# OpenPPL/ppq

Hardware: AMD Instinct MI355X
Metric: calibration samples/sec (RuntimeCalibrationPass, KL 2048-bin, ResNet-50 INT8) (higher is better)
Workload: dtype f32; 1 GPU; ResNet-50 topology (53 Conv + 1 Gemm, BN folded, seeded He init), RuntimeCalibrationPass kl 2048 bins, per-tensor INT8 activations, per-channel INT8 weights, 279 batches x 32 x 3x224x224 per GPU; samples=8928, batch=32, observed_tensors=72, rccl_ranks=1, async_observe=False, cache_params=False, channels_last=False, fuse_params=True, batch_observations=True, reuse_activations=False, replayed_batches=0, hip_graph=auto, graph_replays=0, miopen_find=False

## Files before the change

include/ppq_hip.h:

```cpp
#ifndef PPQ_HIP_H_
#define PPQ_HIP_H_

#include <stdint.h>

#ifdef __cplusplus
extern "C" {
#endif

typedef enum {
    PPQHIP_OK = 0,
    PPQHIP_ERR_INVALID_VALUE = -1,
    PPQHIP_ERR_UNSUPPORTED = -2,
    PPQHIP_ERR_HIP = -3
} ppqhip_status;

#define PPQHIP_ABI_VERSION 4

const char* ppqhip_last_error(void);
int ppqhip_version(void);
int ppqhip_device_arch(char* buf, int n);

int ppqhip_fq_linear_t(const float* x, const float* scale, const float* offset, float* out,
                       int64_t n, int clip_min, int clip_max, int rounding, void* stream);

// ... 191 lines not shown
                         int64_t n, int64_t num_channel, int64_t elem_per_channel,
                         int clip_min, int clip_max, int rounding, void* stream);
int ppqhip_rounding_loss_bwd(const float* x, const float* dy, const float* scale,
                             const float* offset, float* dx, int64_t n, int64_t num_channel,
                             int64_t elem_per_channel, int clip_min, int clip_max, int rounding,
                             void* stream);

int ppqhip_bias_act(float* y, const float* bias, int64_t n, int64_t num_channel, int64_t elem_per_channel,
                    int relu, void* stream);
int ppqhip_bias_add_act(float* a, const float* bias_a, float* b, const float* bias_b, float* out,
                        int64_t n, int64_t num_channel, int64_t elem_per_channel, int relu, void* stream);

#define PPQHIP_NOT_FUSED 1
int ppqhip_bias_act_stats(float* y, const float* bias, int64_t n, int64_t num_channel, int64_t elem_per_channel,
                          int relu, float* slots_y, void* stream);
int ppqhip_bias_add_act_stats(float* a, const float* bias_a, float* b, const float* bias_b, float* out,
                              int64_t n, int64_t num_channel, int64_t elem_per_channel, int relu,
                              float* slots_a, float* slots_b, float* slots_out, void* stream);

#define PPQHIP_ELIDE_A 1
#define PPQHIP_ELIDE_B 2
int ppqhip_bias_add_act_stats2(float* a, const float* bias_a, float* b, const float* bias_b, float* out,
                               int64_t n, int64_t num_channel, int64_t elem_per_channel, int relu,
                               float* slots_a, float* slots_b, float* slots_out, int elide, void* stream);

int ppqhip_bias_act_hist(float* y, const float* bias, int64_t n, int64_t num_channel, int64_t elem_per_channel,
                         int relu, int32_t* rows_y, float p0_y, float p1_y, int64_t num_bins, int asymmetric,
                         int clip_outliers, void* stream);
int ppqhip_bias_add_act_hist(float* a, const float* bias_a, float* b, const float* bias_b, float* out,
                             int64_t n, int64_t num_channel, int64_t elem_per_channel, int relu,
                             int32_t* rows_a, float p0_a, float p1_a, int32_t* rows_b, float p0_b, float p1_b,
                             int32_t* rows_out, float p0_out, float p1_out, int64_t num_bins, int asymmetric,
                             int clip_outliers, int elide, void* stream);

typedef struct ppqhip_adaround_job {
    const float* w;
    const float* v;
    const float* scale;
    const float* offset;
    float* out;
    const float* dy;
    int64_t n, num_channel, elem_per_channel;
    int32_t qmin, qmax;
} ppqhip_adaround_job;
int ppqhip_adaround_fwd_multi(const ppqhip_adaround_job* jobs, int num_jobs, void* stream);
int ppqhip_adaround_bwd_multi(const ppqhip_adaround_job* jobs, int num_jobs, const float* reg, void* stream);

typedef struct ppqhip_roundtune_job {
    const float* w;
    const float* r;
    const float* scale;
    const float* offset;
    float* out;
    int64_t n, num_channel, elem_per_channel;
    int32_t qmin, qmax;
} ppqhip_roundtune_job;
int ppqhip_roundtune_fwd_multi(const ppqhip_roundtune_job* jobs, int num_jobs, void* stream);

typedef struct ppqhip_fetch_rows_job {
    const float* x;
    const int32_t* index;
    float* out;
    int64_t rows, row_len, count;
} ppqhip_fetch_rows_job;
int ppqhip_fetch_rows_multi(const ppqhip_fetch_rows_job* jobs, int num_jobs, void* stream);
typedef struct ppqhip_measure_rows_job {
// ... 169 lines not shown
```

ppq_amd/_lib.py:

```python
import ctypes
import os

_HERE = os.path.dirname(os.path.abspath(__file__))
LIB_PATH = os.path.join(_HERE, 'libppq_hip.so')

c_f32p = ctypes.c_void_p
c_i32p = ctypes.c_void_p
c_f64p = ctypes.c_void_p
c_i64 = ctypes.c_int64
c_int = ctypes.c_int
c_flt = ctypes.c_float
c_vp = ctypes.c_void_p

ABI_VERSION = 4


NOT_FUSED = 1


class ProfEntry(ctypes.Structure):
    _fields_ = [('name', ctypes.c_char * 48), ('launches', ctypes.c_int64),
                ('total_ms', ctypes.c_double), ('total_bytes', ctypes.c_double)]


PROTOTYPES = {
    'ppqhip_last_error': (ctypes.c_char_p, []),
    'ppqhip_version': (c_int, []),
    'ppqhip_device_arch': (c_int, [ctypes.c_char_p, c_int]),
    'ppqhip_fq_linear_t': (c_int, [c_f32p, c_f32p, c_f32p, c_f32p, c_i64, c_int, c_int, c_int, c_vp]),
    'ppqhip_fq_linear_c': (c_int, [c_f32p, c_f32p, c_f32p, c_f32p, c_i64, c_i64, c_i64, c_int, c_int, c_int, c_vp]),
    'ppqhip_to_int_t': (c_int, [c_f32p, c_f32p, c_f32p, c_vp, c_i64, c_int, c_int, c_int, c_int, c_vp]),
    'ppqhip_to_int_c': (c_int, [c_f32p, c_f32p, c_f32p, c_vp, c_i64, c_i64, c_i64, c_int, c_int, c_int, c_int, c_vp]),
    'ppqhip_fq_linear_t_bwd': (c_int, [c_f32p, c_f32p, c_f32p, c_f32p, c_f32p, c_f32p, c_i64, c_int, c_int, c_int,
                                       c_vp]),
    'ppqhip_fq_linear_c_bwd': (c_int, [c_f32p, c_f32p, c_f32p, c_f32p, c_f32p, c_f32p, c_i64, c_i64, c_i64, c_int,
                                       c_int, c_int, c_vp]),
    'ppqhip_fq_linear_c_bwd_multi': (c_int, [c_vp, c_int, c_int, c_vp]),
    'ppqhip_fq_linear_t_bwd_partials': (c_i64, [c_i64]),
    'ppqhip_fq_linear_t_bwd_main': (c_int, [c_f32p, c_f32p, c_f32p, c_f32p, c_f32p, c_f32p, c_i64, c_int, c_int, c_int, c_vp]),
    'ppqhip_lsq_finish_multi': (c_int, [c_vp, c_int, c_vp]),
    'ppqhip_bias_act': (c_int, [c_f32p, c_f32p, c_i64, c_i64, c_i64, c_int, c_vp]),
    'ppqhip_bias_add_act': (c_int, [c_f32p, c_f32p, c_f32p, c_f32p, c_f32p, c_i64, c_i64, c_i64, c_int, c_vp]),
    'ppqhip_bias_act_stats': (c_int, [c_f32p, c_f32p, c_i64, c_i64, c_i64, c_int, c_f32p, c_vp]),
    'ppqhip_bias_add_act_stats': (c_int, [c_f32p, c_f32p, c_f32p, c_f32p, c_f32p, c_i64, c_i64, c_i64, c_int, c_f32p, c_f32p,
                                          c_f32p, c_vp]),
    'ppqhip_bias_add_act_stats2': (c_int, [c_f32p, c_f32p, c_f32p, c_f32p, c_f32p, c_i64, c_i64, c_i64, c_int, c_f32p, c_f32p,
                                           c_f32p, c_int, c_vp]),
    'ppqhip_bias_act_hist': (c_int, [c_f32p, c_f32p, c_i64, c_i64, c_i64, c_int, c_i32p, c_flt, c_flt, c_i64, c_int, c_int, c_vp]),
    'ppqhip_bias_add_act_hist': (c_int, [c_f32p, c_f32p, c_f32p, c_f32p, c_f32p, c_i64, c_i64, c_i64, c_int,
                                         c_i32p, c_flt, c_flt, c_i32p, c_flt, c_flt, c_i32p, c_flt, c_flt, c_i64, c_int, c_int,
                                         c_int, c_vp]),
    'ppqhip_fq_float_t': (c_int, [c_f32p, c_f32p, c_f32p, c_f32p, c_i64, c_int, c_int, c_flt, c_flt, c_int, c_vp]),
    'ppqhip_fq_float_c': (c_int, [c_f32p, c_f32p, c_f32p, c_f32p, c_i64, c_i64, c_i64, c_int, c_int, c_flt, c_flt,
                                  c_int, c_vp]),
    'ppqhip_fq_float_c_bwd': (c_int, [c_f32p, c_f32p, c_f32p, c_f32p, c_f32p, c_f32p, c_i64, c_i64, c_i64, c_int,
                                      c_int, c_flt, c_flt, c_int, c_vp]),
    'ppqhip_hist_workspace_bytes': (c_i64, [c_i64, c_i64]),
    'ppqhip_hist_sym_t': (c_int, [c_f32p, c_i64, c_flt, c_int, c_i32p, c_i64, c_vp, c_vp]),
    'ppqhip_hist_asym_t': (c_int, [c_f32p, c_i64, c_flt, c_flt, c_int, c_i32p, c_i64, c_vp, c_vp]),
    'ppqhip_hist_sym_c': (c_int, [c_f32p, c_i64, c_i64, c_i64, c_flt, c_int, c_i32p, c_i64, c_vp]),
    'ppqhip_hist_sym_c_scales': (c_int, [c_f32p, c_i64, c_i64, c_i64, c_f32p, c_int, c_i32p, c_i64, c_vp]),
    'ppqhip_hist_asym_c_ranges': (c_int, [c_f32p, c_i64, c_i64, c_i64, c_f32p, c_f32p, c_int, c_i32p, c_i64, c_vp]),
    'ppqhip_quantile_workspace_bytes': (c_i64, [c_i64]),
    'ppqhip_quantile_t': (c_int, [c_f32p, c_i64, c_flt, c_f32p, c_vp, c_vp, c_vp]),
    'ppqhip_isotone_t': (c_int, [c_f32p, c_i64, c_f32p, c_vp, c_vp]),
    'ppqhip_minmax_workspace_bytes': (c_i64, [c_i64]),
    'ppqhip_minmax_t': (c_int, [c_f32p, c_i64, c_f32p, c_vp, c_vp]),
    'ppqhip_minmax_c': (c_int, [c_f32p, c_i64, c_i64, c_i64, c_f32p, c_f32p, c_vp]),
    'ppqhip_minmax_c_multi': (c_int, [c_vp, c_int, c_vp]),
    'ppqhip_fq_linear_multi_table_bytes': (c_i64, [c_int]),
    'ppqhip_fq_linear_multi': (c_int, [c_vp, c_int, c_int, c_vp, c_int, c_vp]),
    'ppqhip_float_scale_search_table_bytes': (c_i64, [c_int]),
    'ppqhip_float_scale_search': (c_int, [c_vp, c_int, c_vp, c_int, c_int, c_vp, c_vp, c_vp]),
    'ppqhip_fq_float_multi_table_bytes': (c_i64, [c_int]),
    'ppqhip_fq_float_multi': (c_int, [c_vp, c_int, c_int, c_vp, c_int, c_vp]),
    'ppqhip_quantile_multi_workspace_bytes': (c_i64, [c_int, c_i64]),
    'ppqhip_quantile_t_multi': (c_int, [c_vp, c_int, c_flt, c_vp, c_vp]),
    'ppqhip_quantile_debug_layout': (None, [c_vp]),
    'ppqhip_quantile_hot_layout': (None, [c_vp]),
    'ppqhip_minmax_t_slots_multi': (c_int, [c_vp, c_int, c_vp]),
    'ppqhip_hist_t_rows_multi': (c_int, [c_vp, c_int, c_int, c_int, c_i64, c_vp]),
    'ppqhip_channel_sum': (c_int, [c_f32p, c_i64, c_i64, c_i64, c_f64p, c_vp]),
    'ppqhip_hist_rows': (c_i64, []),
    'ppqhip_hist_sym_t_rows': (c_int, [c_f32p, c_i64, c_flt, c_int, c_i32p, c_i64, c_vp]),
# ... 78 lines not shown
```

ppq_amd/csrc/epilogue.hip:

```cpp
#include "channel_axis.hpp"
#include "common.hpp"
#include "hist_bin.hpp"
#include "minmax_fold.hpp"

namespace ppqhip {
namespace {

constexpr int kEpTileU = 2;
constexpr int kEpSmallU = 1;
constexpr long long kEpSmallElems = 1ll << 20;

struct EpArgs {
    float* a;
    const float* bias_a;
    float* b;
    const float* bias_b;
    float* out;
    uint32_t nvec;
    uint32_t tail;
    int ntail;
    FastDiv epc;
    FastDiv nc;
    uint32_t elide;
};
// ... 390 lines not shown
    uint32_t grid = tiles / kEpHistMinTiles;
    if (grid > cap) grid = cap;
#define PPQ_LAUNCH_EPH(PLANE, ASYM, CLIP)                                                                                 \
    hipLaunchKernelGGL((epilogue_stats_kernel<kEpTileU, RESID, BIAS_B, true, PLANE, EpHistSet<RESID, BIAS_B, ASYM, CLIP>>),  \
                       dim3(grid), dim3(kEpStatBlock), ints * sizeof(int), st, p, sk)
    switch ((plane ? 4 : 0) | (r.asym ? 2 : 0) | (r.clip ? 1 : 0)) {
        case 0: PPQ_LAUNCH_EPH(false, false, false); break;
        case 1: PPQ_LAUNCH_EPH(false, false, true); break;
        case 2: PPQ_LAUNCH_EPH(false, true, false); break;
        case 3: PPQ_LAUNCH_EPH(false, true, true); break;
        case 4: PPQ_LAUNCH_EPH(true, false, false); break;
        case 5: PPQ_LAUNCH_EPH(true, false, true); break;
        case 6: PPQ_LAUNCH_EPH(true, true, false); break;
        default: PPQ_LAUNCH_EPH(true, true, true); break;
    }
#undef PPQ_LAUNCH_EPH
    return finish_launch(what);
}

void set_hist_rule(EpHistSinks& sk, int k, int32_t* rows, float p0, float p1, const EpHistRule& r) {
    sk.rows[k] = rows;
    if (r.asym) { sk.a0[k] = p0; sk.hs[k] = (p1 - p0) / (float)r.bins; }
    else { sk.a0[k] = 0.f; sk.hs[k] = p0; }
}

int validate_elide(const char* what, int elide, bool sink_a, bool sink_b, bool has_bias_b) {
    if (elide & ~(int)(kElideA | kElideB)) { set_error("%s: elide has unknown bits", what); return PPQHIP_ERR_INVALID_VALUE; }
    if (((elide & (int)kElideA) && !sink_a) || ((elide & (int)kElideB) && !(sink_b && has_bias_b))) {
        set_error("%s: a tensor that is not stored needs a sink", what); return PPQHIP_ERR_INVALID_VALUE;
    }
    return PPQHIP_OK;
}

}
}

using namespace ppqhip;

extern "C" {

int ppqhip_bias_act(float* y, const float* bias, int64_t n, int64_t num_channel, int64_t elem_per_channel, int relu,
                    void* stream) {
    if (int st = validate_channel_axis("bias_act", n, num_channel, elem_per_channel)) return st;
    if (!y || !bias) { set_error("bias_act: null pointer"); return PPQHIP_ERR_INVALID_VALUE; }
    hipStream_t s = (hipStream_t)stream;
    EpArgs p{};
    p.a = y; p.bias_a = bias;
    const bool aligned = aligned16(y);
    if (relu) launch_epilogue<false, false, true>(p, n, num_channel, elem_per_channel, aligned, s);
    else launch_epilogue<false, false, false>(p, n, num_channel, elem_per_channel, aligned, s);
    return finish_launch("bias_act");
}

int ppqhip_bias_add_act(float* a, const float* bias_a, float* b, const float* bias_b, float* out, int64_t n,
                        int64_t num_channel, int64_t elem_per_channel, int relu, void* stream) {
    if (int st = validate_channel_axis("bias_add_act", n, num_channel, elem_per_channel)) return st;
    if (!a || !bias_a || !b || !out) { set_error("bias_add_act: null pointer"); return PPQHIP_ERR_INVALID_VALUE; }
    hipStream_t s = (hipStream_t)stream;
    EpArgs p{};
    p.a = a; p.bias_a = bias_a; p.b = b; p.bias_b = bias_b; p.out = out;
    const bool aligned = aligned16(a) && aligned16(b) && aligned16(out);
    if (bias_b) {
        if (relu) launch_epilogue<true, true, true>(p, n, num_channel, elem_per_channel, aligned, s);
        else launch_epilogue<true, true, false>(p, n, num_channel, elem_per_channel, aligned, s);
    } else {
        if (relu) launch_epilogue<true, false, true>(p, n, num_channel, elem_per_channel, aligned, s);
// ... 60 lines not shown
    EpArgs p{};
    p.a = y; p.bias_a = bias;
    return launch_epilogue_hist<false, false>(p, n, num_channel, elem_per_channel, relu, aligned16(y), sk, r, "bias_act_hist",
                                              (hipStream_t)stream);
}

int ppqhip_bias_add_act_hist(float* a, const float* bias_a, float* b, const float* bias_b, float* out, int64_t n,
                             int64_t num_channel, int64_t elem_per_channel, int relu, int32_t* rows_a, float p0_a, float p1_a,
                             int32_t* rows_b, float p0_b, float p1_b, int32_t* rows_out, float p0_out, float p1_out,
                             int64_t num_bins, int asymmetric, int clip_outliers, int elide, void* stream) {
    const char* what = "bias_add_act_hist";
    if (int st = validate_channel_axis(what, n, num_channel, elem_per_channel)) return st;
    if (!a || !bias_a || !b || !out) { set_error("%s: null pointer", what); return PPQHIP_ERR_INVALID_VALUE; }
    if (!bias_b && rows_b) { set_error("%s: without bias_b, b is only read: it has no sink", what); return PPQHIP_ERR_INVALID_VALUE; }
    if (int st = validate_hist_rule(what, num_bins)) return st;
    if (int st = validate_elide(what, elide, rows_a != nullptr, rows_b != nullptr, bias_b != nullptr)) return st;
    if ((rows_a && (rows_a == rows_b || rows_a == rows_out)) || (rows_b && rows_b == rows_out)) {
        set_error("%s: two sinks share one rows accumulator", what); return PPQHIP_ERR_INVALID_VALUE;
    }
    if (num_bins > (int64_t)kEpHistLdsInts) return PPQHIP_NOT_FUSED;
    const EpHistRule r{(int)num_bins, asymmetric ? 1 : 0, clip_outliers ? 1 : 0};
    EpHistSinks sk{};
    set_hist_rule(sk, 0, rows_a, p0_a, p1_a, r);
    set_hist_rule(sk, 1, rows_b, p0_b, p1_b, r);
    set_hist_rule(sk, 2, rows_out, p0_out, p1_out, r);
    EpArgs p{};
    p.a = a; p.bias_a = bias_a; p.b = b; p.bias_b = bias_b; p.out = out; p.elide = (uint32_t)elide;
    const bool aligned = aligned16(a) && aligned16(b) && aligned16(out);
    hipStream_t s = (hipStream_t)stream;
    if (bias_b) return launch_epilogue_hist<true, true>(p, n, num_channel, elem_per_channel, relu, aligned, sk, r, what, s);
    return launch_epilogue_hist<true, false>(p, n, num_channel, elem_per_channel, relu, aligned, sk, r, what, s);
}

}
```

ppq_amd/ffi.py:

```python
import math
import threading
import weakref
from typing import List

import numpy as np
import torch

from . import _lib
from ._lib import lib

_KERNEL_FAILURE = 'Kernel Failure, '


_raw_stream = torch._C._cuda_getCurrentRawStream
_get_device = torch._C._cuda_getDevice


def _stream() -> int:
    return _raw_stream(_get_device())


def _check(t: torch.Tensor, dtype: torch.dtype, name: str) -> None:
    if not isinstance(t, torch.Tensor):
        raise TypeError(f'{name}: expected a torch.Tensor, got {type(t)}')
# ... 112 lines not shown

def _owner_quantile_hint(device: torch.device, numel: int, q: float):
    owner = getattr(_hint_owner, 'current', None)
    if owner is None: return None
    try: per = _owner_hints.setdefault(owner, {})
    except TypeError: return None
    key = (device.index, int(numel), float(q))
    h = per.get(key)
    if h is None: h = per[key] = quantile_hint(device)
    return h


_HIST_JOB = np.dtype([('x', '<u8'), ('rows', '<u8'), ('n', '<i8'), ('p0', '<f4'), ('p1', '<f4')])


def _epilogue_geometry(ts, bias_list):
    t0 = ts[0]
    if not isinstance(t0, torch.Tensor) or t0.dtype is not _F32 or not t0.is_cuda or t0.dim() != 4 or t0.numel() == 0:
        return None
    shape, strides, dev = t0.shape, t0.stride(), t0.device
    for t in ts[1:]:
        if not isinstance(t, torch.Tensor) or t.dtype is not _F32 or t.device != dev or t.shape != shape or t.stride() != strides:
            return None
    C = int(shape[1])
    for bias in bias_list:
        if (not isinstance(bias, torch.Tensor) or bias.dtype is not _F32 or bias.device != dev or bias.dim() != 1
                or bias.numel() != C or not bias.is_contiguous()):
            return None
    if t0.is_contiguous(): return C, int(shape[2]) * int(shape[3])
    if t0.is_contiguous(memory_format=torch.channels_last): return C, 1
    return None


def bias_act_(y: torch.Tensor, bias: torch.Tensor, relu: bool) -> bool:
    geo = _epilogue_geometry([y], [bias])
    if geo is None: return False
    with _DeviceOf(y):
        _raise(lib.ppqhip_bias_act(y.data_ptr(), bias.data_ptr(), y.numel(), geo[0], geo[1], 1 if relu else 0, _stream()))
    return True


def bias_add_act(a: torch.Tensor, bias_a: torch.Tensor, b: torch.Tensor, bias_b, relu: bool):
    geo = _epilogue_geometry([a, b], [bias_a] if bias_b is None else [bias_a, bias_b])
    if geo is None or a.data_ptr() == b.data_ptr(): return None
    out = torch.empty_like(a)
    with _DeviceOf(a):
        _raise(lib.ppqhip_bias_add_act(a.data_ptr(), bias_a.data_ptr(), b.data_ptr(), 0 if bias_b is None else bias_b.data_ptr(),
                                       out.data_ptr(), a.numel(), geo[0], geo[1], 1 if relu else 0, _stream()))
    return out


def _sink_slots(job, dev) -> int:
    if job is None: return 0
    slots = job[1]
    if (job[0] != 'minmax' or slots.dtype is not _F32 or slots.device != dev or not slots.is_contiguous()
            or slots.numel() != 2 * lib.ppqhip_minmax_slots()): raise ValueError('no sink for this job')
    return slots.data_ptr()


def _fused_or_raise(status: int) -> bool:
    if status == _lib.NOT_FUSED: return False
    _raise(status)
    return True


def bias_act_stats_(y: torch.Tensor, bias: torch.Tensor, relu: bool, job) -> bool:
    geo = _epilogue_geometry([y], [bias])
    if geo is None or job is None: return False
    try: slots = _sink_slots(job, y.device)
    except ValueError: return False
    with _DeviceOf(y):
        return _fused_or_raise(lib.ppqhip_bias_act_stats(y.data_ptr(), bias.data_ptr(), y.numel(), geo[0], geo[1],
                                                         1 if relu else 0, slots, _stream()))


ELIDE_A, ELIDE_B = 1, 2


def bias_add_act_stats(a: torch.Tensor, bias_a: torch.Tensor, b: torch.Tensor, bias_b, relu: bool, job_a, job_b, job_out,
                       elide: int = 0):
    geo = _epilogue_geometry([a, b], [bias_a] if bias_b is None else [bias_a, bias_b])
    if geo is None or a.data_ptr() == b.data_ptr(): return None
    if bias_b is None and job_b is not None: return None
    try: slots = [_sink_slots(j, a.device) for j in (job_a, job_b, job_out)]
    except ValueError: return None
    if not any(slots): return None
    out = torch.empty_like(a)
    args = (a.data_ptr(), bias_a.data_ptr(), b.data_ptr(), 0 if bias_b is None else bias_b.data_ptr(), out.data_ptr(),
            a.numel(), geo[0], geo[1], 1 if relu else 0, slots[0], slots[1], slots[2])
    with _DeviceOf(a):
        if elide: ok = _fused_or_raise(lib.ppqhip_bias_add_act_stats2(*args, int(elide), _stream()))
        else: ok = _fused_or_raise(lib.ppqhip_bias_add_act_stats(*args, _stream()))
    return out if ok else None


def _sink_rows(job, dev) -> tuple:
    if job is None: return 0, 0.0, 0.0
    if job[0] != 'hist_rows': raise ValueError('no sink for this job')
    rows = job[1]
    if (rows.dtype is not torch.int32 or rows.device != dev or rows.dim() != 2 or not rows.is_contiguous()
            or rows.shape[0] != lib.ppqhip_hist_rows()): raise ValueError('no sink for this job')
    return rows.data_ptr(), float(job[3]), float(job[4])


def _hist_rule(jobs):
    rules = {(int(j[1].shape[1]), bool(j[2]), bool(j[5])) for j in jobs if j is not None}
    return next(iter(rules)) if len(rules) == 1 else None


def bias_act_hist_(y: torch.Tensor, bias: torch.Tensor, relu: bool, job) -> bool:
    geo = _epilogue_geometry([y], [bias])
    if geo is None or job is None: return False
    try: rows, p0, p1 = _sink_rows(job, y.device)
    except ValueError: return False
    bins, asym, clip = _hist_rule([job])
    with _DeviceOf(y):
        return _fused_or_raise(lib.ppqhip_bias_act_hist(y.data_ptr(), bias.data_ptr(), y.numel(), geo[0], geo[1],
                                                        1 if relu else 0, rows, p0, p1, bins, int(asym), int(clip), _stream()))


def bias_add_act_hist(a: torch.Tensor, bias_a: torch.Tensor, b: torch.Tensor, bias_b, relu: bool, job_a, job_b, job_out,
                      elide: int = 0):
    geo = _epilogue_geometry([a, b], [bias_a] if bias_b is None else [bias_a, bias_b])
    if geo is None or a.data_ptr() == b.data_ptr(): return None
    if bias_b is None and job_b is not None: return None
    try: sinks = [_sink_rows(j, a.device) for j in (job_a, job_b, job_out)]
    except ValueError: return None
    rule = _hist_rule([job_a, job_b, job_out])
    if rule is None: return None
    out = torch.empty_like(a)
    with _DeviceOf(a):
        ok = _fused_or_raise(lib.ppqhip_bias_add_act_hist(
            a.data_ptr(), bias_a.data_ptr(), b.data_ptr(), 0 if bias_b is None else bias_b.data_ptr(), out.data_ptr(),
            a.numel(), geo[0], geo[1], 1 if relu else 0, *sinks[0], *sinks[1], *sinks[2], rule[0], int(rule[1]), int(rule[2]),
            int(elide), _stream()))
    return out if ok else None


_ADAROUND_JOB = np.dtype([('w', '<u8'), ('v', '<u8'), ('scale', '<u8'), ('offset', '<u8'), ('out', '<u8'), ('dy', '<u8'),
                          ('n', '<i8'), ('num_channel', '<i8'), ('elem_per_channel', '<i8'), ('qmin', '<i4'), ('qmax', '<i4')])
_ROUNDTUNE_JOB = np.dtype([('w', '<u8'), ('r', '<u8'), ('scale', '<u8'), ('offset', '<u8'), ('out', '<u8'),
                           ('n', '<i8'), ('num_channel', '<i8'), ('elem_per_channel', '<i8'), ('qmin', '<i4'), ('qmax', '<i4')])


def _weight_map_table(label, dtype, items, outs, dys=None):
    n = len(items)
    if len(outs) != n or (dys is not None and len(dys) != n):
        raise RuntimeError(_KERNEL_FAILURE + f'{label}: argument lists differ in length')
# ... 1717 lines not shown
```

ppq_amd/harness.py:

```python
import contextlib
from typing import Callable, Dict, List, Optional

import torch
import torch.nn.functional as F

from .core import LinearQuantizationConfig, QuantizationStates, TensorQuantizationConfig, is_initial
from .core import QuantizationProperty as P
from .qfunction import PPQuantFunction

PASSIVE_OPERATIONS = {'MaxPool', 'GlobalMaxPool', 'Reshape', 'Flatten', 'Identity', 'Dropout', 'Slice', 'Pad', 'Resize',
                      'Split', 'Transpose', 'Interp', 'Squeeze', 'Unsqueeze'}
COMPUTING_OP = {'Conv', 'Gemm', 'ConvTranspose', 'MatMul'}


class Variable:
    def __init__(self, name: str, value: torch.Tensor = None, is_parameter: bool = False):
        self.name = name
        self.value = value
        self.stored_value = None
        self.is_parameter = is_parameter
        self.dest_ops: List['Operation'] = []
        self.source_op: Optional['Operation'] = None

    def __hash__(self): return hash(self.name)
# ... 89 lines not shown
        self.operations[name] = op
        return out

    def topological_sort(self) -> List[Operation]:
        return list(self.operations.values())


def _forward(op: Operation, x: List[torch.Tensor]):
    t, a = op.type, op.attributes
    if t == 'Conv':
        return F.conv2d(x[0], x[1], x[2] if len(x) > 2 else None, stride=a.get('strides', 1),
                        padding=a.get('pads', 0), groups=a.get('group', 1))
    if t == 'Gemm': return F.linear(x[0], x[1], x[2] if len(x) > 2 else None)
    if t == 'MatMul': return torch.matmul(x[0], x[1])
    if t == 'Relu': return F.relu(x[0])
    if t == 'Gelu': return F.gelu(x[0])
    if t == 'Add': return x[0] + x[1]
    if t == 'MaxPool': return F.max_pool2d(x[0], a['kernel_shape'], a.get('strides', 1), a.get('pads', 0))
    if t == 'GlobalAveragePool': return F.adaptive_avg_pool2d(x[0], 1)
    if t == 'Flatten': return torch.flatten(x[0], 1)
    if t == 'LayerNormalization': return F.layer_norm(x[0], x[0].shape[-1:], x[1], x[2])
    if t == 'Softmax': return F.softmax(x[0], dim=a.get('axis', -1))
    if t == 'Mul': return x[0] * (x[1] if len(x) > 1 else a['value'])
    if t == 'Reshape': return x[0].reshape(a['shape'])
    if t == 'Transpose': return x[0].permute(a['perm'])
    if t == 'Concat': return torch.cat([v.expand(x[-1].shape[0], *v.shape[1:]) if v.shape[0] == 1 else v for v in x],
                                       dim=a.get('axis', 1))
    if t == 'Slice': return x[0].narrow(a['axis'], a['start'], a['length'])
    if t == 'Resize': return F.interpolate(x[0], scale_factor=a.get('scale', 2), mode=a.get('mode', 'nearest'))
    raise NotImplementedError(f'Graph op: {op.name}({op.type}) has no backend implementation')


class EpilogueGroup:
    __slots__ = ('kind', 'ops', 'convs', 'add', 'relu', 'keep')

    def __init__(self, kind, ops, convs, add, relu, keep=()):
        self.kind, self.ops, self.convs, self.add, self.relu, self.keep = kind, ops, convs, add, relu, frozenset(keep)

    def __repr__(self): return f'{self.kind}({", ".join(op.name for op in self.ops)})'


def _in_cfg(op, i):
    return op.config.input_quantization_config[i] if isinstance(op, QuantableOperation) else None


def _out_cfg(op, i):
    return op.config.output_quantization_config[i] if isinstance(op, QuantableOperation) else None


def plan_epilogues(operations: List[Operation], hooks: Dict[str, object] = None, keep=(), passes_through: Callable = None,
                   grad_enabled: bool = False) -> List[EpilogueGroup]:
    if grad_enabled: return []
    from .observer import CalibrationHook
    hooks = hooks or {}
    keep = set(keep)
    if passes_through is None:
        def passes_through(c): return not QuantizationStates.is_activated(c.state)

    def through(*cfgs): return all(c is None or passes_through(c) for c in cfgs)

    def hooks_ok(members, unwritten):
        for op in members:
            h = hooks.get(op.name)
            if h is None: continue
            if type(h) is not CalibrationHook: return False
            if any(c is not None and c in h._observer_table for c in unwritten): return False
        return True

    def conv_ok(op):
        return (op.type == 'Conv' and len(op.inputs) == 3 and op.inputs[2].is_parameter and len(op.outputs) == 1
                and op.outputs[0].name not in keep)

    def only_feeds(v, op): return len(v.dest_ops) == 1 and v.dest_ops[0] is op

    def relu_after(op, i):
        if i >= len(operations): return None
        r = operations[i]
        out = op.outputs[0]
        if r.type != 'Relu' or len(r.inputs) != 1 or r.inputs[0] is not out or not only_feeds(out, r) or out.name in keep:
            return None
        return r

    def try_p2(i):
        for n_conv in (2, 1):
            j = i + n_conv
            if j + 1 >= len(operations): continue
            add, convs = operations[j], operations[i:j]
            if add.type != 'Add' or len(add.inputs) != 2 or len(add.outputs) != 1 or not all(conv_ok(c) for c in convs): continue
            by_out = {c.outputs[0].name: c for c in convs}
            x0, x1 = add.inputs
            if x0.name not in by_out or x0 is x1: continue
            if n_conv == 2 and x1.name not in by_out: continue
            ordered = [by_out[x0.name]] + ([by_out[x1.name]] if n_conv == 2 else [])
            if not all(only_feeds(c.outputs[0], add) for c in convs): continue
            relu = relu_after(add, j + 1)
            if relu is None: continue
            unwritten = (_out_cfg(add, 0), _in_cfg(relu, 0))
            between = [_out_cfg(c, 0) for c in convs] + [_in_cfg(add, 0), _in_cfg(add, 1)]
            if not through(*unwritten, *between): return None
            members = list(operations[i:j + 2])
            if not hooks_ok(members, unwritten): return None
            return EpilogueGroup('P2', members, ordered, add, relu, keep)
        return None

    def try_p1(i):
        conv = operations[i]
        if not conv_ok(conv): return None
        relu = relu_after(conv, i + 1)
        if relu is None: return None
        unwritten = (_out_cfg(conv, 0), _in_cfg(relu, 0))
        if not through(*unwritten) or not hooks_ok([conv, relu], unwritten): return None
        return EpilogueGroup('P1', [conv, relu], [conv], None, relu, keep)

    groups, i = [], 0
    while i < len(operations):
        g = try_p2(i) if operations[i].type == 'Conv' else None
        if g is None and operations[i].type == 'Conv': g = try_p1(i)
        if g is None:
            i += 1
            continue
        groups.append(g)
        i += len(g.ops)
    return groups


def elidable_stores(grp: EpilogueGroup, hooks, jobs: Dict[str, tuple], recorder=None) -> set:
    if grp.kind != 'P2' or recorder is not None or not hooks: return set()
    add_hook = hooks.get(grp.add.name)
    out = set()
    for conv in grp.convs:
        v, hook = conv.outputs[0], hooks.get(conv.name)
        if len(v.dest_ops) != 1 or v.dest_ops[0] is not grp.add or v.name in grp.keep: continue
        if conv.name not in jobs or hook is None or not isinstance(conv, QuantableOperation): continue
        obs = [hook._observer_table.get(c) for c in conv.config.output_quantization_config]
        if len(obs) != 1 or obs[0] is None or not obs[0].reads_only_its_job(): continue
        if add_hook is not None and isinstance(grp.add, QuantableOperation) and any(
                c in add_hook._observer_table for x, c in zip(grp.add.inputs, grp.add.config.input_quantization_config) if x is v):
            continue
        out.add(conv.name)
    return out


class TorchExecutor:
    def __init__(self, graph: BaseGraph, device: str = 'cuda'):
        self._graph = graph
        self._device = device
        self._default_quant_fn = PPQuantFunction
        self.cache_parameter_quantization = False
        self._param_cache: Dict[str, tuple] = {}
        self.fuse_parameter_quantization = True
        self._plans: list = []
        self._plan_signature = None
        self._plan_cache: Dict[tuple, list] = {}
        self._fused: Dict[tuple, torch.Tensor] = {}
        self._delegates: Dict[object, Callable] = {}
        self._overrides: Dict[str, Callable] = {}
        self._takes_packed: set = set()
        self._group_overrides: Dict[str, tuple] = {}
        self.fuse_epilogues = True
        self._epilogue_cache: Dict[tuple, dict] = {}
        self.channels_last = False
        for v in graph.variables.values():
            if v.is_parameter and v.value is not None: v.value = v.value.to(device)

    def use_channels_last(self) -> 'TorchExecutor':
        self.channels_last = True
        for v in self._graph.variables.values():
            if v.is_parameter and isinstance(v.value, torch.Tensor) and v.value.dim() == 4:
                v.value = v.value.contiguous(memory_format=torch.channels_last)
        return self

    def _place(self, value: torch.Tensor) -> torch.Tensor:
# ... 209 lines not shown
                groups = [g for g in groups if not any(m.name in grouped for m in g.ops)]
            plan = {g.ops[0].name: g for g in groups}
            if len(self._epilogue_cache) >= 8: self._epilogue_cache.pop(next(iter(self._epilogue_cache)))
            self._epilogue_cache[sig] = plan
        return plan

    def _run_epilogue(self, grp: EpilogueGroup, raw_of: Callable, hooks) -> Optional[Dict[str, torch.Tensor]]:
        from .ffi import (ELIDE_A, ELIDE_B, bias_act_, bias_act_hist_, bias_act_stats_, bias_add_act, bias_add_act_hist,
                          bias_add_act_stats)
        for conv in grp.convs:
            x, w = raw_of(conv.inputs[0]), conv.inputs[1].value
            if not (isinstance(x, torch.Tensor) and x.is_cuda and x.dtype == torch.float32 and x.dim() == 4
                    and isinstance(w, torch.Tensor) and w.dim() == 4): return None
            fmt = torch.channels_last if self.channels_last else torch.contiguous_format
            if not (x.is_contiguous(memory_format=fmt) and w.is_contiguous(memory_format=fmt)): return None
        if grp.add is not None:
            b_var = grp.add.inputs[1]
            if b_var.source_op not in grp.convs:
                b = raw_of(b_var)
                if not (isinstance(b, torch.Tensor) and b.is_cuda and b.dtype == torch.float32): return None
        hooks = hooks or {}
        ys, biases = {}, {}
        for conv in grp.ops[:len(grp.convs)]:
            qin = self._input_side(conv, [raw_of(v) for v in conv.inputs], hooks.get(conv.name))
            a = conv.attributes
            ys[conv.name] = F.conv2d(qin[0], qin[1], None, stride=a.get('strides', 1), padding=a.get('pads', 0),
                                     groups=a.get('group', 1))
            biases[conv.name] = qin[2]
        if grp.kind == 'P1':
            conv = grp.convs[0]
            y = ys[conv.name]
            stored = {grp.relu.name: y}
            fed = self._epilogue_sinks(grp, hooks, stored, y)
            if fed is not None:
                job = fed[0].get(grp.relu.name)
                launch = bias_act_hist_ if job is not None and job[0] == 'hist_rows' else bias_act_stats_
                if not launch(y, biases[conv.name], True, job): fed = None
            if fed is None and not bias_act_(y, biases[conv.name], relu=True):
                y.add_(biases[conv.name].view(1, -1, 1, 1)).relu_()
            tail, elided = {conv.name: y, grp.relu.name: y}, set()
        else:
            conv_a = grp.convs[0]
            a = ys[conv_a.name]
            conv_b = grp.convs[1] if len(grp.convs) > 1 else None
            b = ys[conv_b.name] if conv_b is not None else raw_of(grp.add.inputs[1])
            bias_b = biases[conv_b.name] if conv_b is not None else None
            stored = {conv_a.name: a, grp.relu.name: None}
            if conv_b is not None: stored[conv_b.name] = b
            fed, out, elided = self._epilogue_sinks(grp, hooks, stored, a), None, set()
            if fed is not None:
                jobs = fed[0]
                elided = elidable_stores(grp, hooks, jobs, fed[1].recorder)
                mask = (ELIDE_A if conv_a.name in elided else 0) | (ELIDE_B if conv_b is not None and conv_b.name in elided else 0)
                launch = bias_add_act_hist if next(iter(jobs.values()))[0] == 'hist_rows' else bias_add_act_stats
                out = launch(a, biases[conv_a.name], b, bias_b, True, jobs.get(conv_a.name),
                             jobs.get(conv_b.name) if conv_b is not None else None, jobs.get(grp.relu.name), mask)
                if out is None: fed, elided = None, set()
                else: stored[grp.relu.name] = out
            if out is None: out = bias_add_act(a, biases[conv_a.name], b, bias_b, relu=True)
            if out is None:
                a.add_(biases[conv_a.name].view(1, -1, 1, 1))
                if conv_b is not None: b.add_(biases[conv_b.name].view(1, -1, 1, 1))
                out = F.relu(a + b)
            tail = {conv_a.name: a, grp.add.name: out, grp.relu.name: out}
            if conv_b is not None: tail[conv_b.name] = b
        if fed is not None:
            for name, job in fed[0].items(): fed[1].prepay(stored[name], job[1])
        values: Dict[str, torch.Tensor] = {}
        for op in grp.ops:
            hook = hooks.get(op.name)
            if op.type != 'Conv':
                self._input_side(op, [values[v.name] if v.name in values else raw_of(v) for v in op.inputs], hook)
            for v, y in zip(op.outputs, self._output_side(op, tail[op.name], hook)): values[v.name] = y
        for name in elided:
            for v in next(m for m in grp.ops if m.name == name).outputs: values[v.name] = None
        return values

    @ staticmethod
    def _epilogue_sinks(grp: EpilogueGroup, hooks, stored: Dict[str, torch.Tensor], like: torch.Tensor):
        jobs, queue = {}, None
        for op in grp.ops:
            hook = hooks.get(op.name)
            if hook is None or not isinstance(op, QuantableOperation): continue
            for cfg in op.config.output_quantization_config:
                ob = hook._observer_table.get(cfg)
                if ob is None: continue
                if op.name not in stored or op.name in jobs or hook.stream is not None or ob.queue is None: return None
                if queue is not None and ob.queue is not queue: return None
                job = ob.stat_job(like)
                if job is None: return None
                jobs[op.name], queue = job, ob.queue
        if len({job[0] for job in jobs.values()}) > 1: return None
        return (jobs, queue) if jobs else None

    def _quantize_parameter(self, var: Variable, config) -> torch.Tensor:
        hit = self._fused.get((var.name, id(config)))
        if hit is not None: return hit
        if not self.cache_parameter_quantization or not QuantizationStates.is_activated(config.state):
            return self.quantize_function(var.value, config)
        key = (var.value.data_ptr(), var.value._version, id(config.scale), config.scale._version,
               id(config.offset), config.offset._version, int(getattr(config.state, 'value', config.state)))
        hit = self._param_cache.get(var.name)
        if hit is not None and hit[0] == key: return hit[1]
        q = self.quantize_function(var.value, config)
        self._param_cache[var.name] = (key, q)
# ... 339 lines not shown
```

Baseline: 3810 samples/s.

## Fuse stem MaxPool into conv bias+ReLU epilogue with optional stats/hist sinks

Adds HIP kernels that apply bias and ReLU to a conv output, stage each plane in LDS, and compute the following MaxPool directly. Min/max or histogram observation can be fed in the same pass. The harness now groups Conv+Relu+MaxPool and can skip storing the ReLU output when only the pool reads it. This is meant to remove a separate pooling kernel launch and an extra read/write of the large stem activation. In exchange it constrains fusion to whole planes fitting in LDS, which may limit occupancy.

```diff
diff --git a/include/ppq_hip.h b/include/ppq_hip.h
--- a/include/ppq_hip.h
+++ b/include/ppq_hip.h
@@ -247,6 +247,17 @@
                              int32_t* rows_a, float p0_a, float p1_a, int32_t* rows_b, float p0_b, float p1_b,
                              int32_t* rows_out, float p0_out, float p1_out, int64_t num_bins, int asymmetric,
                              int clip_outliers, int elide, void* stream);
+
+int ppqhip_bias_act_pool(float* y, const float* bias, float* pool, int64_t n, int64_t num_channel, int64_t height,
+                         int64_t width, int relu, int kernel, int stride, int pad, int dilation, int ceil_mode,
+                         void* stream);
+int ppqhip_bias_act_pool_stats(float* y, const float* bias, float* pool, int64_t n, int64_t num_channel, int64_t height,
+                               int64_t width, int relu, int kernel, int stride, int pad, int dilation, int ceil_mode,
+                               float* slots_y, int store_relu, void* stream);
+int ppqhip_bias_act_pool_hist(float* y, const float* bias, float* pool, int64_t n, int64_t num_channel, int64_t height,
+                              int64_t width, int relu, int kernel, int stride, int pad, int dilation, int ceil_mode,
+                              int32_t* rows_y, float p0_y, float p1_y, int64_t num_bins, int asymmetric,
+                              int clip_outliers, int store_relu, void* stream);
 
 typedef struct ppqhip_adaround_job {
     const float* w;
diff --git a/ppq_amd/_lib.py b/ppq_amd/_lib.py
--- a/ppq_amd/_lib.py
+++ b/ppq_amd/_lib.py
@@ -50,6 +50,12 @@
     'ppqhip_bias_add_act_hist': (c_int, [c_f32p, c_f32p, c_f32p, c_f32p, c_f32p, c_i64, c_i64, c_i64, c_int,
                                          c_i32p, c_flt, c_flt, c_i32p, c_flt, c_flt, c_i32p, c_flt, c_flt, c_i64, c_int, c_int,
                                          c_int, c_vp]),
+    'ppqhip_bias_act_pool': (c_int, [c_f32p, c_f32p, c_f32p, c_i64, c_i64, c_i64, c_i64, c_int, c_int, c_int, c_int, c_int, c_int,
+                                     c_vp]),
+    'ppqhip_bias_act_pool_stats': (c_int, [c_f32p, c_f32p, c_f32p, c_i64, c_i64, c_i64, c_i64, c_int, c_int, c_int, c_int, c_int,
+                                           c_int, c_f32p, c_int, c_vp]),
+    'ppqhip_bias_act_pool_hist': (c_int, [c_f32p, c_f32p, c_f32p, c_i64, c_i64, c_i64, c_i64, c_int, c_int, c_int, c_int, c_int,
+                                          c_int, c_i32p, c_flt, c_flt, c_i64, c_int, c_int, c_int, c_vp]),
     'ppqhip_fq_float_t': (c_int, [c_f32p, c_f32p, c_f32p, c_f32p, c_i64, c_int, c_int, c_flt, c_flt, c_int, c_vp]),
     'ppqhip_fq_float_c': (c_int, [c_f32p, c_f32p, c_f32p, c_f32p, c_i64, c_i64, c_i64, c_int, c_int, c_flt, c_flt,
                                   c_int, c_vp]),
diff --git a/ppq_amd/csrc/epilogue.hip b/ppq_amd/csrc/epilogue.hip
--- a/ppq_amd/csrc/epilogue.hip
+++ b/ppq_amd/csrc/epilogue.hip
@@ -446,6 +446,203 @@
     return PPQHIP_OK;
 }
 
+struct EpNoSinks {
+    struct Args {};
+    __device__ __forceinline__ void init(const Args&, int*) {}
+    __device__ __forceinline__ void begin() {}
+    template <bool FULL>
+    __device__ __forceinline__ void feed4(const EpStored<float4>&, bool, bool) {}
+    __device__ __forceinline__ void finish(const Args&, uint32_t, int*) {}
+};
+
+constexpr uint32_t kEpPoolStage = 2 * kWave;
+constexpr uint32_t kEpPoolStageBytes = (kEpStatBlock / kWave) * kEpPoolStage * sizeof(float);
+constexpr uint32_t kEpPoolMaxLds = 64u * 1024u;
+constexpr int kEpPoolMaxKernel = 3;
+
+struct EpPoolArgs {
+    float* y;
+    const float* bias;
+    float* pool;
+    uint32_t planes;
+    uint32_t hw4;
+    uint32_t H, W, ohw;
+    int k, s, pad;
+    FastDiv nc;
+    FastDiv ow;
+    uint32_t store;
+    uint32_t vec;
+    uint32_t sink_ints;
+};
+
+__device__ __forceinline__ void lds_barrier() {
+    asm volatile("s_waitcnt lgkmcnt(0)\n\ts_barrier" ::: "memory");
+}
+
+__device__ __forceinline__ float pool_at(const float* plane, const EpPoolArgs& p, uint32_t o) {
+    const uint32_t oh = fdiv(o, p.ow), ow = o - oh * p.ow.d;
+    const int h0 = (int)oh * p.s - p.pad, w0 = (int)ow * p.s - p.pad;
+    float v[kEpPoolMaxKernel][kEpPoolMaxKernel];
+#pragma unroll
+    for (int kh = 0; kh < kEpPoolMaxKernel; kh++) {
+        const int ih = h0 + kh;
+        const bool row = kh < p.k && (uint32_t)ih < p.H;
+        const uint32_t first = (uint32_t)min(max(ih, 0), (int)p.H - 1) * p.W;
+#pragma unroll
+        for (int kw = 0; kw < kEpPoolMaxKernel; kw++) {
+            const int iw = w0 + kw;
+            const float t = plane[first + (uint32_t)min(max(iw, 0), (int)p.W - 1)];
+            v[kh][kw] = (row && kw < p.k && (uint32_t)iw < p.W) ? t : -INFINITY;
+        }
+    }
+    float m = -INFINITY;
+#pragma unroll
+    for (int kh = 0; kh < kEpPoolMaxKernel; kh++)
+#pragma unroll
+        for (int kw = 0; kw < kEpPoolMaxKernel; kw++)
+            if (v[kh][kw] > m || __builtin_isnan(v[kh][kw])) m = v[kh][kw];
+    return m;
+}
+
+template <int U, bool RELU, class SINKS>
+__global__ __launch_bounds__(kEpStatBlock, (kEpStatBlock * kEpStatWgPerCu + 255) / 256)
+void epilogue_pool_kernel(EpPoolArgs p, typename SINKS::Args sk) {
+    extern __shared__ int lds[];
+    constexpr uint32_t kTile = (uint32_t)kEpStatBlock * U;
+    float* plane = reinterpret_cast<float*>(lds + p.sink_ints);
+    float4* plane4 = reinterpret_cast<float4*>(plane);
+    float* stage = plane + p.hw4 * 4u + (threadIdx.x >> 6) * kEpPoolStage;
+    float4* y4 = reinterpret_cast<float4*>(p.y);
+    uint32_t pl, pl_end;
+    even_split(p.planes, gridDim.x, blockIdx.x, pl, pl_end);
+    const uint32_t steps = (p.hw4 + kTile - 1) / kTile;
+    SINKS sinks;
+    sinks.init(sk, lds);
+
+    struct Tile { float4 a[U]; float bias; };
+    auto fetch = [&](Tile& T, uint32_t pi, uint32_t step) {
+        const uint32_t first = pi * p.hw4, base = step * kTile + threadIdx.x;
+#pragma unroll
+        for (int u = 0; u < U; u++) T.a[u] = y4[first + min(base + u * kEpStatBlock, p.hw4 - 1)];
+        T.bias = p.bias[pi - fdiv(pi, p.nc) * p.nc.d];
+    };
+    auto pool_plane = [&](uint32_t pi) {
+        float* dst = p.pool + (size_t)pi * p.ohw;
+        const uint32_t lane = threadIdx.x & 63, wave_first = (threadIdx.x >> 6) * kEpPoolStage;
+        for (uint32_t base = 0; base < p.ohw; base += (kEpStatBlock / kWave) * kEpPoolStage) {
+            const uint32_t o0 = base + wave_first + lane, o1 = o0 + kWave;
+            const float m0 = o0 < p.ohw ? pool_at(plane, p, o0) : 0.f;
+            const float m1 = o1 < p.ohw ? pool_at(plane, p, o1) : 0.f;
+            if (p.vec) {
+                stage[lane] = m0;
+                stage[kWave + lane] = m1;
+                __builtin_amdgcn_fence(__ATOMIC_RELEASE, "wavefront");
+                __builtin_amdgcn_wave_barrier();
+                const uint32_t o4 = base + wave_first + 4u * lane;
+                if (lane < kEpPoolStage / 4 && o4 < p.ohw)
+                    *reinterpret_cast<float4*>(dst + o4) = *reinterpret_cast<const float4*>(stage + 4u * lane);
+                __builtin_amdgcn_fence(__ATOMIC_ACQ_REL, "wavefront");
+                __builtin_amdgcn_wave_barrier();
+            } else {
+                if (o0 < p.ohw) dst[o0] = m0;
+                if (o1 < p.ohw) dst[o1] = m1;
+            }
+        }
+    };
+    auto consume = [&](const Tile& T, uint32_t pi, uint32_t step) {
+        const uint32_t first = pi * p.hw4, base = step * kTile + threadIdx.x;
+        const float4 bias = make_float4(T.bias, T.bias, T.bias, T.bias);
+        const bool full = (step + 1) * kTile <= p.hw4;
+        EpStored<float4> s[U];
+        bool in[U];
+#pragma unroll
+        for (int u = 0; u < U; u++) {
+            const uint32_t vv = base + u * kEpStatBlock;
+            in[u] = vv < p.hw4;
+            s[u] = EpStored<float4>{};
+            s[u].a = act4<RELU>(add4(T.a[u], bias));
+            if (in[u]) {
+                if (p.store) y4[first + vv] = s[u].a;
+                plane4[vv] = s[u].a;
+            }
+        }
+        if (full) {
+#pragma unroll
+            for (int u = 0; u < U; u++) sinks.template feed4<true>(s[u], true, u == 0);
+        } else {
+#pragma unroll
+            for (int u = 0; u < U; u++)
+                if (__builtin_amdgcn_ballot_w64(in[u]) != 0ull) sinks.template feed4<false>(s[u], in[u], true);
+        }
+        if (step + 1 == steps) {
+            lds_barrier();
+            pool_plane(pi);
+            lds_barrier();
+        }
+    };
+    uint32_t cp = pl, cs = 0;
+    Tile ta{}, tb{};
+    fetch(ta, cp, cs);
+    sinks.begin();
+    for (;;) {
+        uint32_t np = cp, ns = cs + 1;
+        if (ns == steps) { ns = 0; np++; }
+        bool last = np >= pl_end;
+        fetch(tb, last ? cp : np, last ? cs : ns);
+        consume(ta, cp, cs);
+        if (last) break;
+        cp = np; cs = ns;
+        ns = cs + 1;
+        if (ns == steps) { ns = 0; np++; }
+        last = np >= pl_end;
+        fetch(ta, last ? cp : np, last ? cs : ns);
+        consume(tb, cp, cs);
+        if (last) break;
+        cp = np; cs = ns;
+    }
+    sinks.finish(sk, blockIdx.x, lds);
+}
+
+int fill_pool_geometry(EpPoolArgs& p, int64_t n, int64_t C, int64_t H, int64_t W, int kernel, int stride, int pad, int dilation,
+                       int ceil_mode, uint32_t sink_ints, uint32_t& lds_bytes) {
+    if (kernel < 1 || kernel > kEpPoolMaxKernel || stride < 1 || pad < 0 || 2 * pad > kernel || dilation != 1 || ceil_mode != 0)
+        return PPQHIP_NOT_FUSED;
+    const int64_t hw = H * W;
+    if (hw % 4 != 0 || H + 2 * pad < kernel || W + 2 * pad < kernel || !aligned16(p.y) || !aligned16(p.pool)) return PPQHIP_NOT_FUSED;
+    const int64_t OH = (H + 2 * pad - kernel) / stride + 1, OW = (W + 2 * pad - kernel) / stride + 1, planes = n / hw;
+    if (planes * OH * OW > 0x7fffffffLL) return PPQHIP_NOT_FUSED;
+    sink_ints = (sink_ints + 3u) & ~3u;
+    const int64_t bytes = (int64_t)sink_ints * 4 + hw * 4 + kEpPoolStageBytes;
+    if (bytes > (int64_t)kEpPoolMaxLds) return PPQHIP_NOT_FUSED;
+    lds_bytes = (uint32_t)bytes;
+    p.planes = (uint32_t)planes; p.hw4 = (uint32_t)(hw / 4);
+    p.H = (uint32_t)H; p.W = (uint32_t)W; p.ohw = (uint32_t)(OH * OW);
+    p.k = kernel; p.s = stride; p.pad = pad;
+    p.nc = make_fastdiv((uint32_t)C); p.ow = make_fastdiv((uint32_t)OW);
+    p.vec = p.ohw % 4u == 0 ? 1u : 0u;
+    p.sink_ints = sink_ints;
+    return PPQHIP_OK;
+}
+
+uint32_t pool_grid(const EpPoolArgs& p) {
+    const uint32_t cap = (uint32_t)(num_cu() * kEpStatWgPerCu);
+    return p.planes < cap ? p.planes : cap;
+}
+
+int validate_pool(const char* what, const float* y, const float* bias, const float* pool, int64_t n, int64_t C, int64_t H, int64_t W) {
+    if (H <= 0 || W <= 0 || H > 0x7fffffffLL || W > 0x7fffffffLL || H * W > 0x7fffffffLL) {
+        set_error("%s: the plane %lld x %lld is empty or too large", what, (long long)H, (long long)W); return PPQHIP_ERR_INVALID_VALUE;
+    }
+    if (int st = validate_channel_axis(what, n, C, H * W)) return st;
+    if (!y || !bias || !pool) { set_error("%s: null pointer", what); return PPQHIP_ERR_INVALID_VALUE; }
+    return PPQHIP_OK;
+}
+
+int validate_pool_store(const char* what, int store_relu, bool sink) {
+    if (!store_relu && !sink) { set_error("%s: a tensor that is not stored needs a sink", what); return PPQHIP_ERR_INVALID_VALUE; }
+    return PPQHIP_OK;
+}
+
 }
 }
 
@@ -572,4 +769,67 @@
     return launch_epilogue_hist<true, false>(p, n, num_channel, elem_per_channel, relu, aligned, sk, r, what, s);
 }
 
-}
+#define PPQ_LAUNCH_POOL(RELU, SET, SK)                                                                                    \
+    hipLaunchKernelGGL((epilogue_pool_kernel<kEpTileU, RELU, SET>), dim3(pool_grid(p)), dim3(kEpStatBlock), lds_bytes,      \
+                       (hipStream_t)stream, p, SK)
+
+int ppqhip_bias_act_pool(float* y, const float* bias, float* pool, int64_t n, int64_t num_channel, int64_t height, int64_t width,
+                         int relu, int kernel, int stride, int pad, int dilation, int ceil_mode, void* stream) {
+    const char* what = "bias_act_pool";
+    if (int st = validate_pool(what, y, bias, pool, n, num_channel, height, width)) return st;
+    EpPoolArgs p{};
+    p.y = y; p.bias = bias; p.pool = pool; p.store = 1u;
+    uint32_t lds_bytes = 0;
+    if (int st = fill_pool_geometry(p, n, num_channel, height, width, kernel, stride, pad, dilation, ceil_mode, 0, lds_bytes)) return st;
+    const EpNoSinks::Args sk{};
+    if (relu) PPQ_LAUNCH_POOL(true, EpNoSinks, sk); else PPQ_LAUNCH_POOL(false, EpNoSinks, sk);
+    return finish_launch(what);
+}
+
+int ppqhip_bias_act_pool_stats(float* y, const float* bias, float* pool, int64_t n, int64_t num_channel, int64_t height,
+                               int64_t width, int relu, int kernel, int stride, int pad, int dilation, int ceil_mode,
+                               float* slots_y, int store_relu, void* stream) {
+    const char* what = "bias_act_pool_stats";
+    if (int st = validate_pool(what, y, bias, pool, n, num_channel, height, width)) return st;
+    if (int st = validate_pool_store(what, store_relu, slots_y != nullptr)) return st;
+    if (!slots_y) return PPQHIP_NOT_FUSED;
+    EpPoolArgs p{};
+    p.y = y; p.bias = bias; p.pool = pool; p.store = store_relu ? 1u : 0u;
+    uint32_t lds_bytes = 0;
+    if (int st = fill_pool_geometry(p, n, num_channel, height, width, kernel, stride, pad, dilation, ceil_mode, 32, lds_bytes)) return st;
+    const EpMinMaxSinks sk{{slots_y, nullptr, nullptr}};
+    using Set = EpMinMaxSet<false, false>;
+    if (relu) PPQ_LAUNCH_POOL(true, Set, sk); else PPQ_LAUNCH_POOL(false, Set, sk);
+    return finish_launch(what);
+}
+
+int ppqhip_bias_act_pool_hist(float* y, const float* bias, float* pool, int64_t n, int64_t num_channel, int64_t height,
+                              int64_t width, int relu, int kernel, int stride, int pad, int dilation, int ceil_mode,
+                              int32_t* rows_y, float p0_y, float p1_y, int64_t num_bins, int asymmetric, int clip_outliers,
+                              int store_relu, void* stream) {
+    const char* what = "bias_act_pool_hist";
+    if (int st = validate_pool(what, y, bias, pool, n, num_channel, height, width)) return st;
+    if (int st = validate_hist_rule(what, num_bins)) return st;
+    if (int st = validate_pool_store(what, store_relu, rows_y != nullptr)) return st;
+    if (!rows_y || !relu || num_bins > (int64_t)kEpHistLdsInts) return PPQHIP_NOT_FUSED;
+    const EpHistRule r{(int)num_bins, asymmetric ? 1 : 0, clip_outliers ? 1 : 0};
+    EpHistSinks sk{};
+    set_hist_rule(sk, 0, rows_y, p0_y, p1_y, r);
+    sk.lds_ints = (uint32_t)r.bins; sk.bins = r.bins;
+    EpPoolArgs p{};
+    p.y = y; p.bias = bias; p.pool = pool; p.store = store_relu ? 1u : 0u;
+    uint32_t lds_bytes = 0;
+    if (int st = fill_pool_geometry(p, n, num_channel, height, width, kernel, stride, pad, dilation, ceil_mode, sk.lds_ints, lds_bytes)) return st;
+#define PPQ_LAUNCH_POOLH(ASYM, CLIP) { using Set = EpHistSet<false, false, ASYM, CLIP>; PPQ_LAUNCH_POOL(true, Set, sk); }
+    switch ((r.asym ? 2 : 0) | (r.clip ? 1 : 0)) {
+        case 0: PPQ_LAUNCH_POOLH(false, false); break;
+        case 1: PPQ_LAUNCH_POOLH(false, true); break;
+        case 2: PPQ_LAUNCH_POOLH(true, false); break;
+        default: PPQ_LAUNCH_POOLH(true, true); break;
+    }
+#undef PPQ_LAUNCH_POOLH
+    return finish_launch(what);
+}
+#undef PPQ_LAUNCH_POOL
+
+}
diff --git a/ppq_amd/ffi.py b/ppq_amd/ffi.py
--- a/ppq_amd/ffi.py
+++ b/ppq_amd/ffi.py
@@ -168,8 +168,24 @@
     return None
 
 
-def bias_act_(y: torch.Tensor, bias: torch.Tensor, relu: bool) -> bool:
+def _pool_launch(y: torch.Tensor, geo, pool):
+    k, s, p = (int(v) for v in pool)
+    if geo is None or not y.is_contiguous() or k < 1 or s < 1 or p < 0: return None
+    N, C, H, W = (int(v) for v in y.shape)
+    if H + 2 * p < k or W + 2 * p < k: return None
+    pooled = torch.empty((N, C, (H + 2 * p - k) // s + 1, (W + 2 * p - k) // s + 1), dtype=_F32, device=y.device)
+    return pooled, (y.numel(), C, H, W), (k, s, p, 1, 0)
+
+
+def bias_act_(y: torch.Tensor, bias: torch.Tensor, relu: bool, pool=None):
     geo = _epilogue_geometry([y], [bias])
+    if pool is not None:
+        args = _pool_launch(y, geo, pool)
+        if args is None: return None
+        with _DeviceOf(y):
+            ok = _fused_or_raise(lib.ppqhip_bias_act_pool(y.data_ptr(), bias.data_ptr(), args[0].data_ptr(), *args[1],
+                                                          1 if relu else 0, *args[2], _stream()))
+        return args[0] if ok else None
     if geo is None: return False
     with _DeviceOf(y):
         _raise(lib.ppqhip_bias_act(y.data_ptr(), bias.data_ptr(), y.numel(), geo[0], geo[1], 1 if relu else 0, _stream()))
@@ -200,11 +216,18 @@
     return True
 
 
-def bias_act_stats_(y: torch.Tensor, bias: torch.Tensor, relu: bool, job) -> bool:
+def bias_act_stats_(y: torch.Tensor, bias: torch.Tensor, relu: bool, job, pool=None, store: bool = True):
     geo = _epilogue_geometry([y], [bias])
-    if geo is None or job is None: return False
+    if geo is None or job is None: return None if pool is not None else False
     try: slots = _sink_slots(job, y.device)
-    except ValueError: return False
+    except ValueError: return None if pool is not None else False
+    if pool is not None:
+        args = _pool_launch(y, geo, pool)
+        if args is None: return None
+        with _DeviceOf(y):
+            ok = _fused_or_raise(lib.ppqhip_bias_act_pool_stats(y.data_ptr(), bias.data_ptr(), args[0].data_ptr(), *args[1],
+                                                                1 if relu else 0, *args[2], slots, 1 if store else 0, _stream()))
+        return args[0] if ok else None
     with _DeviceOf(y):
         return _fused_or_raise(lib.ppqhip_bias_act_stats(y.data_ptr(), bias.data_ptr(), y.numel(), geo[0], geo[1],
                                                          1 if relu else 0, slots, _stream()))
@@ -244,12 +267,20 @@
     return next(iter(rules)) if len(rules) == 1 else None
 
 
-def bias_act_hist_(y: torch.Tensor, bias: torch.Tensor, relu: bool, job) -> bool:
+def bias_act_hist_(y: torch.Tensor, bias: torch.Tensor, relu: bool, job, pool=None, store: bool = True):
     geo = _epilogue_geometry([y], [bias])
-    if geo is None or job is None: return False
+    if geo is None or job is None: return None if pool is not None else False
     try: rows, p0, p1 = _sink_rows(job, y.device)
-    except ValueError: return False
+    except ValueError: return None if pool is not None else False
     bins, asym, clip = _hist_rule([job])
+    if pool is not None:
+        args = _pool_launch(y, geo, pool)
+        if args is None: return None
+        with _DeviceOf(y):
+            ok = _fused_or_raise(lib.ppqhip_bias_act_pool_hist(y.data_ptr(), bias.data_ptr(), args[0].data_ptr(), *args[1],
+                                                               1 if relu else 0, *args[2], rows, p0, p1, bins, int(asym), int(clip),
+                                                               1 if store else 0, _stream()))
+        return args[0] if ok else None
     with _DeviceOf(y):
         return _fused_or_raise(lib.ppqhip_bias_act_hist(y.data_ptr(), bias.data_ptr(), y.numel(), geo[0], geo[1],
                                                         1 if relu else 0, rows, p0, p1, bins, int(asym), int(clip), _stream()))
diff --git a/ppq_amd/harness.py b/ppq_amd/harness.py
--- a/ppq_amd/harness.py
+++ b/ppq_amd/harness.py
@@ -145,12 +145,26 @@
 
 
 class EpilogueGroup:
-    __slots__ = ('kind', 'ops', 'convs', 'add', 'relu', 'keep')
-
-    def __init__(self, kind, ops, convs, add, relu, keep=()):
+    __slots__ = ('kind', 'ops', 'convs', 'add', 'relu', 'keep', 'pool')
+
+    def __init__(self, kind, ops, convs, add, relu, keep=(), pool=None):
         self.kind, self.ops, self.convs, self.add, self.relu, self.keep = kind, ops, convs, add, relu, frozenset(keep)
+        self.pool = pool
 
     def __repr__(self): return f'{self.kind}({", ".join(op.name for op in self.ops)})'
+
+
+def pool_window(op: Operation) -> Optional[tuple]:
+    a = op.attributes
+
+    def square(value):
+        if isinstance(value, (list, tuple)):
+            if not 1 <= len(value) <= 2 or any(v != value[0] for v in value): return None
+            value = value[0]
+        return value if isinstance(value, int) and not isinstance(value, bool) else None
+    if 'kernel_shape' not in a or square(a.get('dilations', 1)) != 1 or a.get('ceil_mode', 0) not in (0, False): return None
+    window = tuple(square(v) for v in (a['kernel_shape'], a.get('strides', 1), a.get('pads', 0)))
+    return None if any(v is None for v in window) else window
 
 
 def _in_cfg(op, i):
@@ -193,6 +207,15 @@
         if r.type != 'Relu' or len(r.inputs) != 1 or r.inputs[0] is not out or not only_feeds(out, r) or out.name in keep:
             return None
         return r
+
+    def pool_after(relu, i):
+        if i >= len(operations): return None
+        m, out = operations[i], relu.outputs[0]
+        if (m.type != 'MaxPool' or len(m.inputs) != 1 or len(m.outputs) != 1 or m.inputs[0] is not out or not only_feeds(out, m)
+                or out.name in keep or pool_window(m) is None): return None
+        between = (_out_cfg(relu, 0), _in_cfg(m, 0))
+        if not through(*between) or not hooks_ok([m], between[1:]): return None
+        return m
 
     def try_p2(i):
         for n_conv in (2, 1):
@@ -223,7 +246,8 @@
         if relu is None: return None
         unwritten = (_out_cfg(conv, 0), _in_cfg(relu, 0))
         if not through(*unwritten) or not hooks_ok([conv, relu], unwritten): return None
-        return EpilogueGroup('P1', [conv, relu], [conv], None, relu, keep)
+        pool = pool_after(relu, i + 2)
+        return EpilogueGroup('P1', [conv, relu] + ([pool] if pool is not None else []), [conv], None, relu, keep, pool)
 
     groups, i = [], 0
     while i < len(operations):
@@ -238,19 +262,22 @@
 
 
 def elidable_stores(grp: EpilogueGroup, hooks, jobs: Dict[str, tuple], recorder=None) -> set:
-    if grp.kind != 'P2' or recorder is not None or not hooks: return set()
-    add_hook = hooks.get(grp.add.name)
+    if recorder is not None or not hooks: return set()
+    if grp.kind == 'P2': producers, reader = grp.convs, grp.add
+    elif grp.pool is not None: producers, reader = [grp.relu], grp.pool
+    else: return set()
+    reader_hook = hooks.get(reader.name)
     out = set()
-    for conv in grp.convs:
-        v, hook = conv.outputs[0], hooks.get(conv.name)
-        if len(v.dest_ops) != 1 or v.dest_ops[0] is not grp.add or v.name in grp.keep: continue
-        if conv.name not in jobs or hook is None or not isinstance(conv, QuantableOperation): continue
-        obs = [hook._observer_table.get(c) for c in conv.config.output_quantization_config]
+    for op in producers:
+        v, hook = op.outputs[0], hooks.get(op.name)
+        if len(v.dest_ops) != 1 or v.dest_ops[0] is not reader or v.name in grp.keep: continue
+        if op.name not in jobs or hook is None or not isinstance(op, QuantableOperation): continue
+        obs = [hook._observer_table.get(c) for c in op.config.output_quantization_config]
         if len(obs) != 1 or obs[0] is None or not obs[0].reads_only_its_job(): continue
-        if add_hook is not None and isinstance(grp.add, QuantableOperation) and any(
-                c in add_hook._observer_table for x, c in zip(grp.add.inputs, grp.add.config.input_quantization_config) if x is v):
+        if reader_hook is not None and isinstance(reader, QuantableOperation) and any(
+                c in reader_hook._observer_table for x, c in zip(reader.inputs, reader.config.input_quantization_config) if x is v):
             continue
-        out.add(conv.name)
+        out.add(op.name)
     return out
 
 
@@ -526,13 +553,22 @@
             y = ys[conv.name]
             stored = {grp.relu.name: y}
             fed = self._epilogue_sinks(grp, hooks, stored, y)
+            window = pool_window(grp.pool) if grp.pool is not None and not self.channels_last else None
+            pooled, elided = None, set()
             if fed is not None:
                 job = fed[0].get(grp.relu.name)
                 launch = bias_act_hist_ if job is not None and job[0] == 'hist_rows' else bias_act_stats_
-                if not launch(y, biases[conv.name], True, job): fed = None
-            if fed is None and not bias_act_(y, biases[conv.name], relu=True):
-                y.add_(biases[conv.name].view(1, -1, 1, 1)).relu_()
-            tail, elided = {conv.name: y, grp.relu.name: y}, set()
+                if window is not None:
+                    elided = elidable_stores(grp, hooks, fed[0], fed[1].recorder)
+                    pooled = launch(y, biases[conv.name], True, job, pool=window, store=not elided)
+                    if pooled is None: elided = set()
+                if pooled is None and not launch(y, biases[conv.name], True, job): fed = None
+            if fed is None:
+                if window is not None: pooled = bias_act_(y, biases[conv.name], relu=True, pool=window)
+                if pooled is None and not bias_act_(y, biases[conv.name], relu=True):
+                    y.add_(biases[conv.name].view(1, -1, 1, 1)).relu_()
+            tail = {conv.name: y, grp.relu.name: y}
+            if grp.pool is not None: tail[grp.pool.name] = pooled
         else:
             conv_a = grp.convs[0]
             a = ys[conv_a.name]
@@ -564,7 +600,8 @@
         for op in grp.ops:
             hook = hooks.get(op.name)
             if op.type != 'Conv':
-                self._input_side(op, [values[v.name] if v.name in values else raw_of(v) for v in op.inputs], hook)
+                qin = self._input_side(op, [values[v.name] if v.name in values else raw_of(v) for v in op.inputs], hook)
+                if tail[op.name] is None: tail[op.name] = _forward(op, qin)
             for v, y in zip(op.outputs, self._output_side(op, tail[op.name], hook)): values[v.name] = y
         for name in elided:
             for v in next(m for m in grp.ops if m.name == name).outputs: values[v.name] = None
```

Result: faster. 3856 samples/s, median of 6 (+1.2%).
